# woolgathering/pyPeriod

Hardware: AMD Instinct MI355X
Metric: window-projections/sec (all-p sweep, N=4096) (higher is better)
Workload: dtype f64

## Files before the change

pyperiod_amd/csrc/period_hip.hip:

```cpp
#include <hip/hip_runtime.h>

#include <algorithm>
#include <cstdarg>
#include <cstdio>
#include <cstdlib>
#include <cstring>
#include <string>
#include <vector>

#include "../../include/periodhip.h"
#include "ph_kernels.h"
#include "ph_fit.h"
#include "ph_frames.h"

namespace {

thread_local std::string g_err;

int fail(int code, const char* fmt, ...) {
  char buf[512];
  va_list ap;
  va_start(ap, fmt);
  vsnprintf(buf, sizeof buf, fmt, ap);
  va_end(ap);
// ... 1391 lines not shown
  PH_TRY(st.out(B_OUT2, bases, (size_t)W * num * N * sz, &dbases));
  PH_TRY(st.out(B_OUT3, status, (size_t)W * sizeof(int32_t), &dstat));
  void* dsweeps;
  PH_TRY(st.out(B_OUT4, n_sweeps, (size_t)W * sizeof(int32_t), &dsweeps));
  PH_TRY(ensure(c, c->buf[B_WS0], (size_t)W * sizeof(double)));
  double* dnorm = static_cast<double*>(c->buf[B_WS0].p);
  const int row_stride = (max_length + 127) & ~127;
  PH_TRY(ensure(c, c->buf[B_WS1], (size_t)W * num * row_stride * sz));
  void* drows = c->buf[B_WS1].p;
  const unsigned kflags = flags & (PH_FLAG_TRUNC | PH_FLAG_ORTH);
  const int max_iters = 12 * (P + num) + 64;
  const dim3 grid((unsigned)W);
  if (pair) {
    PairWs ws;
    PH_TRY(pair_workspace(c, W, N, &ws));
    PH_TRY(launch(c, "k_mbest_step1", ph::k_mbest_step1_pair, dim3((unsigned)((W + 1) / 2)), s1.block, s1.lds,
                  (const double*)dx, (int)W, N, num, min_length, max_length, p_scr, gamma, tb.fac_off, tb.fac_q, geom, ws.geomf,
                  ws.radq, plan, n_pass, ws.gwin, max_iters, (uint32_t*)dper, (double*)dpow, (double*)drows, row_stride, dnorm,
                  (int*)dstat, (int*)dsweeps, c->pair_fold_once ? ph::pair_thin_band(N) : -1.0, c->pair_fold_report ? 1 : 0));
  } else {
    PH_TRY(dispatch(dtype, !gwin1, [&](auto t, auto lw) {
      using T = decltype(t);
      return launch(c, "k_mbest_step1", ph::k_mbest_step1<T, decltype(lw)::value>, grid, s1.block, s1.lds, (const T*)dx, N,
                    num, min_length, max_length, gamma, kflags, tb, geom, plan, n_pass, (T*)gbuf1, (T*)gwin1, max_iters,
                    (uint32_t*)dper, (double*)dpow, (T*)drows, row_stride, dnorm, (int*)dstat, (int*)dsweeps,
                    s1.small_means);
    }));
  }
  PH_TRY(dispatch(dtype, !gwin2, [&](auto t, auto lw) {
    using T = decltype(t);
    return launch(c, "k_mbest_step2", ph::k_mbest_step2<T, decltype(lw)::value>, grid, s2.block, s2.lds, N, num, gamma,
                  max_length, kflags, tb, geom, max_fac, (T*)gbuf2, (T*)gwin2, (uint32_t*)dper, (double*)dpow, (T*)dbases,
                  dnorm, (const int*)dstat, (T*)drows, row_stride);
  }));
// ... 1094 lines not shown
```

pyperiod_amd/csrc/ph_device.h:

```cpp
#pragma once

#include <hip/hip_runtime.h>
#include <stdint.h>

#include <type_traits>

namespace ph {

constexpr int kWave = 64;
constexpr int kBlock = 256;
constexpr int kBlockWide = 512;
constexpr int kMaxWaves = 16;
constexpr int kPairWaves = 16;

constexpr unsigned kTrunc = 1u;
constexpr unsigned kOrth = 2u;
constexpr unsigned kSingle = 4u;

struct Tables {
  const int* orth_off;
  const int* orth_q;
  const int* fac_off;
  const int* fac_q;
};
// ... 146 lines not shown
  a = uniform_f64(ta);
  b = uniform_f64(tb);
}

template <int NW = 0>
__device__ __forceinline__ double block_max(double v, double* red) {
  const int tid = threadIdx.x;
  const int nw = wave_count<NW>();
  v = wave_max(v);
  if ((tid & (kWave - 1)) == 0) red[tid >> 6] = v;
  __syncthreads();
  const double t = red_combine<true, NW>(red, nw);
  __syncthreads();
  return uniform_f64(t);
}

struct Fold {
  int p;
  int rows;
  int nfull;
  int trows;
  __device__ __forceinline__ Fold(int N, int p_) : p(p_) {
    rows = (N + p_ - 1) / p_;
    const int shortn = rows * p_ - N;
    nfull = p_ - shortn;
    trows = shortn == 0 ? rows : rows - 1;
  }
  __device__ __forceinline__ Fold(int p_, int rows_, int nfull_) : p(p_), rows(rows_), nfull(nfull_), trows(nfull_ == p_ ? rows_ : rows_ - 1) {}
  __device__ __forceinline__ int count(int j) const { return j < nfull ? rows : rows - 1; }
};
// ... 677 lines not shown
  take(v, p, dpp_f64<kDppRor8>(v), __builtin_amdgcn_update_dpp(0, p, kDppRor8, 0xF, 0xF, false));
  take(v, p, dpp_f64<kDppHalfMirror>(v), __builtin_amdgcn_update_dpp(0, p, kDppHalfMirror, 0xF, 0xF, false));
  take(v, p, dpp_f64<kDppXor2>(v), __builtin_amdgcn_update_dpp(0, p, kDppXor2, 0xF, 0xF, false));
  take(v, p, dpp_f64<kDppXor1>(v), __builtin_amdgcn_update_dpp(0, p, kDppXor1, 0xF, 0xF, false));
}

template <typename T>
__device__ __forceinline__ double block_sweep_value(const T* __restrict__ xs, T* __restrict__ buf, int N, int p,
                                                    int gamma_div, unsigned flags, const Tables& tb,
                                                    double* red) {
  project_lds(xs, buf, N, p, flags, tb);
  const double ss = block_sumsq(buf, N, red);
  return periodic_norm_from_sq(ss, N, gamma_div);
}

template <typename T>
__device__ __forceinline__ void zero_pad(T* __restrict__ xs, int N) {
  for (int i = threadIdx.x; i < kPad; i += blockDim.x) xs[N + i] = T(0);
}

template <typename T>
__device__ __forceinline__ void load_window(const T* __restrict__ g, T* __restrict__ xs, int N) {
  constexpr int V = 16 / sizeof(T);
  if ((reinterpret_cast<uintptr_t>(g) & 15) == 0 && (N % V) == 0) {
    using vec_t = typename std::conditional<sizeof(T) == 8, double2, float4>::type;
    const vec_t* gv = reinterpret_cast<const vec_t*>(g);
    vec_t* xv = reinterpret_cast<vec_t*>(xs);
    for (int i = threadIdx.x; i < N / V; i += blockDim.x) xv[i] = gv[i];
  } else {
    for (int i = threadIdx.x; i < N; i += blockDim.x) xs[i] = g[i];
  }
}

struct Carve {
  unsigned char* base;
  size_t off;
  __device__ explicit Carve(unsigned char* b) : base(b), off(0) {}
  template <typename U>
  __device__ U* take(size_t n) {
    U* p = reinterpret_cast<U*>(base + off);
    off += (n * sizeof(U) + 15) & ~size_t(15);
    return p;
  }
  __device__ Carve at(size_t o) const {
    Carve c(base);
// ... 113 lines not shown
```

pyperiod_amd/csrc/ph_mbest.h:

```cpp
#pragma once

#include "ph_device.h"
#include "ph_pair.h"

namespace ph {

__device__ __forceinline__ bool skip_test(const uint32_t* skip, int i) { return (skip[i >> 5] >> (i & 31)) & 1u; }
__device__ __forceinline__ void skip_set(uint32_t* skip, int i) { skip[i >> 5] |= 1u << (i & 31); }

template <typename Norm>
__device__ __forceinline__ bool mbest_prefers(double ss, int p, double best_ss, int bestp, int gamma, Norm&& norm) {
  bool take = bestp == 0;
  if (!take) {
    const double lhs = gamma ? ss * (double)bestp : ss;
    const double rhs = gamma ? best_ss * (double)p : best_ss;
    if (lhs > rhs * (1.0 + 1e-14)) {
      take = true;
    } else if (lhs >= rhs * (1.0 - 1e-14)) {
      const double vn = norm(ss, gamma ? p : 0);
      const double vb = norm(best_ss, gamma ? bestp : 0);
      take = vn > vb || (vn == vb && p < bestp);
    }
  }
  return take;
// ... 221 lines not shown
constexpr int kPairCoop = 6;

enum {
  MP_LISTED = 0,
  MP_FILLED = 2,
  MP_REPEATS = 4,
  MP_STATUS = 6,
  MP_SWEEPS = 8,
  MP_RUNNING = 10,
  MP_EXACT_ALL = 12,
  MP_QUEUE = 14,
  MP_WORDS = 16
};
enum { MP_UNIT = 0, MP_SCALE = 2, MP_DOUBLES = 4 };

__device__ __forceinline__ double pair_exact_part(const double* __restrict__ xs, int p, const PGeom& g, int first, int stride) {
  double part = 0.0;
  for (int j = first; j < p; j += stride) {
    const bool full = j < g.nfull;
    const double s = column_sum(xs, j, p, full ? g.rows : g.rows - 1);
    part = fma(s * s, full ? g.w_full : g.w_short, part);
  }
  return part;
}

struct Step1PairLds {
  f2* pw;
  double* stg;
  double* red;
  double* wbest;
  int* wbestp;
  double* norms;
  uint32_t* periods;
  uint32_t* skip;
  int* list;
  int* ctl;
  double* dst2;
  double* msm;
  double* prt;
  size_t bytes;
};
template <class C>
__host__ __device__ __forceinline__ Step1PairLds step1_pair_carve(C cv, int N, int num, int P) {
  Step1PairLds L;
  L.pw = cv.template take<f2>(N + kPad);
  L.stg = cv.template take<double>(N + kPad);
  L.red = cv.template take<double>(kRedDoubles);
  L.wbest = cv.template take<double>(kMaxWaves);
  L.wbestp = cv.template take<int>(kMaxWaves);
  L.norms = cv.template take<double>(2 * num);
  L.periods = cv.template take<uint32_t>(2 * num);
  L.skip = cv.template take<uint32_t>(2 * ((P + 31) / 32));
  L.list = cv.template take<int>(2 * kPairListCap);
  L.ctl = cv.template take<int>(MP_WORDS);
  L.dst2 = cv.template take<double>(MP_DOUBLES);
  L.msm = cv.template take<double>(kPairSmallP);
  L.prt = cv.template take<double>(kPairSplitW);
  L.bytes = cv.off;
  return L;
}

__global__ __launch_bounds__(1024) __attribute__((amdgpu_waves_per_eu(PH_STEP1_WAVES, 8))) void k_mbest_step1_pair(
    const double* __restrict__ x, int W, int N, int num, int p_lo, int p_hi, int p_scr, int gamma,
    const int* __restrict__ fac_off, const int* __restrict__ fac_q, const PGeom* __restrict__ geom, const PGeomF* __restrict__ geomf, const double* __restrict__ radq, const PassPlan* __restrict__ plan, int n_pass,
    double* __restrict__ gres, int max_iters, uint32_t* __restrict__ periods_out, double* __restrict__ norms_out,
    double* __restrict__ rows_out, int row_stride, double* __restrict__ dnorm_out, int* __restrict__ status_out,
    int* __restrict__ sweeps_out, double thin_band, int fold_report) {
  const bool fold_once = __double2hiint(thin_band) >= 0;
  extern __shared__ __attribute__((aligned(16))) unsigned char smem[];
  const int P = p_hi - p_lo + 1;
  const int SK = (P + 31) / 32;
  const Step1PairLds L = step1_pair_carve(Carve(smem), N, num, P);
  f2* pw = L.pw;
  double *stg = L.stg, *red = L.red, *wbest = L.wbest, *norms = L.norms, *dst2 = L.dst2, *msm = L.msm, *prt = L.prt;
  int *wbestp = L.wbestp, *list = L.list, *ctl = L.ctl;
  uint32_t *periods = L.periods, *skip = L.skip;

  const int tid = threadIdx.x;
  const int wv = __builtin_amdgcn_readfirstlane(tid >> 6);
  constexpr int NW = kPairWaves, nw = NW;
  const size_t gstride = win_stride((size_t)N);
  float* pwf = reinterpret_cast<float*>(pw);
  const double sqrtN = uniform_f64(sqrt((double)N));

  for (int k = tid; k < 2 * num; k += blockDim.x) {
    norms[k] = 0.0;
    periods[k] = 0u;
  }
  for (int k = tid; k < 2 * SK; k += blockDim.x) skip[k] = 0u;
  if (tid < MP_WORDS) ctl[tid] = tid == MP_QUEUE ? nw : 0;
  zero_pad(stg, N);
  for (int i = tid; i < kPad; i += blockDim.x) pw[N + i] = f2_zero();
  for (int w = 0; w < 2; ++w) {
    const int64_t gw = 2 * (int64_t)blockIdx.x + w;
    const bool exists = gw < W;
    __syncthreads();
    if (exists) {
      load_window(x + gw * (int64_t)N, stg, N);
    } else {
      for (int n = tid; n < N; n += blockDim.x) stg[n] = 0.0;
    }
    __syncthreads();
    const double rsq = block_sumsq<NW>(stg, N, red);
    const double sc = uniform_f64(pair_pick_scale(rsq, N));
    for (int n = tid; n < N; n += blockDim.x) pwf[2 * n + w] = (float)(stg[n] * sc);
    if (tid == 0) {
      dst2[MP_UNIT + w] = rsq * sc * sc * (1.0 + 1e-9);
      dst2[MP_SCALE + w] = sc;
      ctl[MP_RUNNING + w] = exists ? 1 : 0;
      ctl[MP_EXACT_ALL + w] = pair_usable(rsq) ? 0 : 1;
      if (exists) dnorm_out[gw] = periodic_norm_from_sq_n(rsq, sqrtN, 0);
    }
  }
  StageClock<kPairTimers, 6, 3> clk;
  WgStamp<kClocks> stamp;
  for (;;) {
    __syncthreads();
    const bool act0 = __builtin_amdgcn_readfirstlane(ctl[MP_RUNNING]) != 0, act1 = __builtin_amdgcn_readfirstlane(ctl[MP_RUNNING + 1]) != 0;
    if (!act0 && !act1) break;
    prio_by_progress(__builtin_amdgcn_readfirstlane(max(ctl[MP_SWEEPS], ctl[MP_SWEEPS + 1])));
    if (wv == 0 && pair_lane() == 0) ctl[MP_LISTED] = ctl[MP_LISTED + 1] = 0;
    f2* vals = reinterpret_cast<f2*>(stg);
    pair_sweep_plan<false, true>(
        pw, N, geomf, plan, wv, n_pass, nw, [&](float z, int q) { pair_store1(vals, z, q, p_lo); },
        [&](float z, int q_a, int q_b) { pair_store2(vals, z, q_a, q_b, p_lo); },
        PH_PAIR_QUEUE ? &ctl[MP_QUEUE] : nullptr);
    __syncthreads();
    clk.mark(0);
    prio_short_phase();
    {
    const int tid = (wv << 6) + pair_lane();
    const int lane = tid & (kWave - 1);
    if (tid == 0) ctl[MP_QUEUE] = nw;
    {
      const bool scr0 = act0 && !__builtin_amdgcn_readfirstlane(ctl[MP_EXACT_ALL]), scr1 = act1 && !__builtin_amdgcn_readfirstlane(ctl[MP_EXACT_ALL + 1]);
      if (scr0 || scr1) {
        const double unit0 = uniform_f64(dst2[MP_UNIT]), unit1 = uniform_f64(dst2[MP_UNIT + 1]);
        const int i0 = p_scr - p_lo;
        const bool cover = i0 > 0;
        const int SD = (i0 + 31) >> 5;
        uint32_t* seen = reinterpret_cast<uint32_t*>(stg);
        for (int k = tid; k < 2 * SD; k += blockDim.x) seen[k] = 0u;
        const double slack = cover ? pair_cover_slack(N) : 0.0;
        struct Entry {
          f2 v;
          double rad, rq;
          bool skip0, skip1;
        };
        auto entry = [&](int idx) {
          Entry e;
          const int q = p_lo + idx;
          const uint32_t bit = 1u << (idx & 31);
          e.v = vals[idx];
          e.rad = radq[q];
          e.rq = gamma ? 1.0 / (double)q : 1.0;
          e.skip0 = (skip[idx >> 5] & bit) != 0;
          e.skip1 = (skip[SK + (idx >> 5)] & bit) != 0;
          return e;
        };
        const int idx_own = i0 + tid;
        Entry own = {f2_zero(), 0.0, 1.0, true, true};
        if (idx_own < P) own = entry(idx_own);
        const double ninf = const_at_use(-1.0 / 0.0);
        double lo0 = ninf, lo1 = ninf;
        for (int idx = idx_own; idx < P; idx += blockDim.x) {
          const Entry e = idx == idx_own ? own : entry(idx);
          double a = (double)e.v.x - e.rad * unit0, b = (double)e.v.y - e.rad * unit1;
          if (gamma) {
            a *= e.rq;
            b *= e.rq;
          }
          if (!e.skip0 && a > lo0) lo0 = a;
          if (!e.skip1 && b > lo1) lo1 = b;
        }
        lo0 = wave_max(lo0);
        lo1 = wave_max(lo1);
        if (lane == 0) {
          red[wv] = lo0;
          red[kMaxWaves + wv] = lo1;
        }
        __syncthreads();
        lo0 = uniform_f64(red_combine<true, NW>(red, nw));
        lo1 = uniform_f64(red_combine<true, NW>(red + kMaxWaves, nw));
        const bool none0 = cover && scr0 && !(lo0 > ninf), none1 = cover && scr1 && !(lo1 > ninf);
        if (tid == 0 && none0) ctl[MP_LISTED] = kPairListCap + 1;
        if (tid == 0 && none1) ctl[MP_LISTED + 1] = kPairListCap + 1;
        const double thr0 = lo0 - fabs(lo0) * 1e-9, thr1 = lo1 - fabs(lo1) * 1e-9;
        for (int idx = idx_own; idx < P; idx += blockDim.x) {
          const Entry e = idx == idx_own ? own : entry(idx);
          const int q = p_lo + idx;
          const double rad = e.rad + slack;
          double a = (double)e.v.x + rad * unit0, b = (double)e.v.y + rad * unit1;
          if (gamma) {
            a *= e.rq;
            b *= e.rq;
          }
          const bool hit0 = scr0 && !none0 && a >= thr0, hit1 = scr1 && !none1 && b >= thr1;
          if (hit0 && !e.skip0) {
            const int k = atomicAdd(&ctl[MP_LISTED], 1);
            if (k < kPairListCap) list[k] = q;
          }
          if (hit1 && !e.skip1) {
            const int k = atomicAdd(&ctl[MP_LISTED + 1], 1);
// ... 9 lines not shown
              for (int w = 0; w < 2; ++w) {
                if (!(w ? hit1 : hit0) || (skip[w * SK + (di >> 5)] & dbit)) continue;
                if (atomicOr(&seen[w * SD + (di >> 5)], dbit) & dbit) continue;
                const int k = atomicAdd(&ctl[MP_LISTED + w], 1);
                if (k < kPairListCap) list[w * kPairListCap + k] = d;
              }
            }
          }
        }
      }
    }
    __syncthreads();
    clk.mark(1);
    for (int w = 0; w < 2; ++w) {
      if (!(w ? act1 : act0)) continue;
      const int64_t gw = 2 * (int64_t)blockIdx.x + w;
      int filled = __builtin_amdgcn_readfirstlane(ctl[MP_FILLED + w]), repeats = __builtin_amdgcn_readfirstlane(ctl[MP_REPEATS + w]), status = 0,
          iters = __builtin_amdgcn_readfirstlane(ctl[MP_SWEEPS + w]);
      const int nlisted = __builtin_amdgcn_readfirstlane(ctl[MP_LISTED + w]);
      const bool exact_all = __builtin_amdgcn_readfirstlane(ctl[MP_EXACT_ALL + w]) != 0 || nlisted > kPairListCap;
      int ncand = exact_all ? P : nlisted;
      double* nrm = norms + w * num;
      uint32_t* per = periods + w * num;
      uint32_t* sk = skip + w * SK;
      const int* lst = list + w * kPairListCap;
      __syncthreads();
      bool folded = false;
      if (iters + 1 > max_iters) {
        status = 2;
      } else {
// ... 6 lines not shown
          const int q0 = k0 < ncand ? lst[k0] : 0, q1 = k1 < ncand ? lst[k1] : 0;
          const unsigned long long t0 = __ballot(q0 >= p_scr), t1 = __ballot(q1 >= p_scr);
          if (__popcll(t0) + __popcll(t1) == 1) {
            const int m = t0 ? __builtin_amdgcn_readlane(q0, __builtin_amdgcn_readfirstlane(__ffsll((long long)t0) - 1))
                             : __builtin_amdgcn_readlane(q1, __builtin_amdgcn_readfirstlane(__ffsll((long long)t1) - 1));
            const float fm = (float)m;
            const int c0 = (int)(fm * __builtin_amdgcn_rcpf((float)max(q0, 1)) + 0.5f), c1 = (int)(fm * __builtin_amdgcn_rcpf((float)max(q1, 1)) + 0.5f);
            const bool odd = (k0 < ncand && c0 * q0 != m) || (k1 < ncand && c1 * q1 != m);
            if (m > kPairSmallP && __ballot(odd) == 0ull) fold_m = m;
          }
        }
        if (fold_m != 0) {
          const PGeom gm = geom[fold_m];
          double part = 0.0;
          if (tid == 0) wbestp[0] = 0;
          for (int j = tid; j < fold_m; j += blockDim.x) {
            const bool full = j < gm.nfull;
            const double s = pair_column_sum_global(src, j, fold_m, full ? gm.rows : gm.rows - 1);
            part = fma(s * s, full ? gm.w_full : gm.w_short, part);
            stg[j] = s;
          }
          fold_ss = block_sum<NW>(part, red);
          clk.mark(2);
          if (ncand > 1) {
            const int se = __builtin_amdgcn_frexp_exp(dst2[MP_SCALE + w]) - 1;
            const double band = thin_band * ldexp(dst2[MP_UNIT + w], -2 * se);
            double tie = 1e-9;
            asm volatile("" : "+s"(tie));
            const double thr = fold_ss - fabs(fold_ss) * tie - band;
            for (int k = wv; k < ncand; k += nw) {
              const int d = __builtin_amdgcn_readfirstlane(lst[k]);
              if (d == fold_m) continue;
              const double t = wave_sum(pair_thin_part(stg, fold_m, d, geom[d], lane));
              if (lane == 0 && !(t < thr)) wbestp[0] = 1;
            }
            __syncthreads();
            if (__builtin_amdgcn_readfirstlane(wbestp[0]) != 0) fold_m = 0;
          }
          clk.mark(3);
        }
        if (fold_m == 0) {
        load_window(src, stg, N);
        __syncthreads();
        clk.mark(2);
        if (p_scr > p_lo && !exact_all && ncand > 1) {
          for (int k = wv; k < ncand; k += nw) {
            const int p = lst[k];
            const PGeom g = geom[p];
            const double part = p < 64 ? wave_partial_small(stg, N, p, g, lane) : pair_exact_part(stg, p, g, lane, kWave);
            const double ss = wave_sum(part);
            if (lane == 0) msm[k] = ss;
          }
          __syncthreads();
          if (wv == 0) {
            const int k0 = lane, k1 = kWave + lane;
            const double v0 = k0 < ncand ? msm[k0] : -1.0, v1 = k1 < ncand ? msm[k1] : -1.0;
            const int q0 = lst[k0], q1 = k1 < kPairListCap ? lst[k1] : 0;
// ... 21 lines not shown
          clk.count(2, fold_m != 0 ? 1 : 0);
        }
        double best_ss = 0.0;
        int bestp = 0;
        const auto norm = [&](double s, int div) { return periodic_norm_from_sq_n(s, sqrtN, div); };
        auto consider = [&](double ss, int p) {
          if (!(ss > 0.0)) return;
          if (mbest_prefers(ss, p, best_ss, bestp, gamma, norm)) {
            best_ss = ss;
            bestp = p;
          }
        };
        double best = 0.0;
        if (fold_m != 0) {
          consider(fold_ss, fold_m);
          best = bestp != 0 ? periodic_norm_from_sq_n(best_ss, sqrtN, gamma ? bestp : 0) : 0.0;
          if (!(best > 0.0)) bestp = 0;
        } else if (ncand <= kPairCoop) {
          for (int k = 0; k < ncand; ++k) {
            const int p = exact_all ? p_lo + k : lst[k];
            if (skip_test(sk, p - p_lo)) continue;
            const PGeom g = geom[p];
            double part = 0.0;
            if (p < 64) {
              if (wv == 0) part = wave_partial_small(stg, N, p, g, lane);
            } else {
              part = pair_exact_part(stg, p, g, tid, blockDim.x);
            }
            consider(block_sum<NW>(part, red), p);
          }
          best = bestp != 0 ? periodic_norm_from_sq_n(best_ss, sqrtN, gamma ? bestp : 0) : 0.0;
          if (!(best > 0.0)) bestp = 0;
        } else {
          for (int k = wv; k < ncand; k += nw) {
            const int p = exact_all ? p_lo + k : lst[k];
            if (skip_test(sk, p - p_lo)) continue;
            const PGeom g = geom[p];
            const double part = p < 64 ? wave_partial_small(stg, N, p, g, lane) : pair_exact_part(stg, p, g, lane, kWave);
            consider(wave_sum(part), p);
          }
          best = bestp != 0 ? periodic_norm_from_sq_n(best_ss, sqrtN, gamma ? bestp : 0) : 0.0;
          if (!(best > 0.0)) bestp = 0;
// ... 11 lines not shown
        } else {
          int row = -1;
          for (int k0 = 0; k0 < num; k0 += kWave) {
            const unsigned long long hit = __ballot(k0 + lane < num && per[k0 + lane] == (uint32_t)bestp);
            if (hit) row = k0 + 63 - __clzll(hit);
          }
          const int action = mbest_book(row, bestp, best, p_lo, tid, filled, repeats, nrm, per, sk);
          double* brow = rows_out + (gw * (int64_t)num + (row < 0 ? 0 : row)) * row_stride;
          const bool more = filled < num;
          const double sc = uniform_f64(dst2[MP_SCALE + w]);
          double* dst = gres + gw * gstride;
          double acc = 0.0;
          const PGeom gb = geom[__builtin_amdgcn_readfirstlane(bestp)];
          const Fold f(bestp, gb.rows, gb.nfull);
          if (fold_m != 0) {
            for (int j = tid; j < bestp; j += blockDim.x) {
              const int cnt = f.count(j);
              const double m = stg[j] / (double)cnt;
              if (action == 1)
                brow[j] = m;
              else if (action == 2)
                brow[j] += m;
              if (more) {
                for (int r0 = 0; r0 < cnt; r0 += 4) {
                  const unsigned at = (unsigned)(r0 * bestp + j);
                  double v[4];
#pragma unroll
                  for (int u = 0; u < 4; ++u) v[u] = src[r0 + u < cnt ? at + (unsigned)(u * bestp) : at];
#pragma unroll
                  for (int u = 0; u < 4; ++u) {
                    if (r0 + u < cnt) {
// ... 6 lines not shown
                  }
                }
              }
            }
          } else if (bestp <= kPairSmallP) {
            split_row_means(stg, msm, prt, N, bestp, tid, kPairSplitW);
            if (tid < bestp) {
              const double m = msm[tid];
              if (action == 1)
                brow[tid] = m;
              else if (action == 2)
                brow[tid] += m;
            }
            if (more) {
              int idx = tid % bestp;
              const int step = blockDim.x % bestp;
              for (int n = tid; n < N; n += blockDim.x) {
                const double v = stg[n] - msm[idx];
                dst[n] = v;
                pwf[2 * n + w] = (float)(v * sc);
                acc = fma(v, v, acc);
                idx += step;
                idx = idx >= bestp ? idx - bestp : idx;
              }
            }
          } else {
            for (int j = tid; j < bestp; j += blockDim.x) {
              const double m = residue_mean(stg, f, j, false);
              const int cnt = f.count(j);
              if (action == 1)
                brow[j] = m;
              else if (action == 2)
                brow[j] += m;
              if (more) {
                for (int r = 0; r < cnt; ++r) {
                  const int n = r * bestp + j;
                  const double v = stg[n] - m;
                  dst[n] = v;
                  pwf[2 * n + w] = (float)(v * sc);
                  acc = fma(v, v, acc);
                }
              }
            }
          }
          if (more) {
            const double rsq = block_sum<NW>(acc, red);
            const double unit = rsq * sc * sc;
            const bool ok = rsq > 0.0 && rsq < const_at_use(1.79e308);
            if (ok && unit < const_at_use(kPairStaleMeanSq) * (double)const_at_use(N)) {
              const double sc2 = uniform_f64(pair_pick_scale(rsq, N));
              __syncthreads();
              pair_rescale(pwf, w, N, (float)(sc2 / sc), tid);
              if (tid == 0) {
                dst2[MP_UNIT + w] = rsq * sc2 * sc2 * (1.0 + 1e-9);
                dst2[MP_SCALE + w] = sc2;
              }
            } else if (tid == 0) {
              dst2[MP_UNIT + w] = unit * (1.0 + 1e-9);
            }
            if (tid == 0) ctl[MP_EXACT_ALL + w] = ok ? 0 : 1;
          }
        }
      }
      __syncthreads();
      if (tid == 0) {
        ctl[MP_FILLED + w] = filled;
        ctl[MP_REPEATS + w] = repeats;
        ctl[MP_STATUS + w] = status | (((ctl[MP_STATUS + w] >> 8) + (folded ? 1 : 0)) << 8);
        ctl[MP_SWEEPS + w] = iters;
        ctl[MP_RUNNING + w] = (status == 0 && filled < num) ? 1 : 0;
      }
      clk.mark(5);
    }
    }
  }
  if (kClocks && (blockIdx.x % 16) == 7 && tid == 0) {
    stamp.finish();
    printf("PAIRWG %d start %lld end %lld cycles %lld MHz %.0f hwid %x xcc %x\n", (int)blockIdx.x, stamp.wk0, stamp.wk1, stamp.ck1 - stamp.ck0,
           100.0 * (double)(stamp.ck1 - stamp.ck0) / (double)(stamp.wk1 - stamp.wk0), stamp.hwid, stamp.xcc);
  }
  if (kPairTimers && blockIdx.x < PH_PAIR_TIMERS_WGS && tid == 0)
    printf("pair timers (100 MHz ticks) screen %lld scan %lld load %lld thin %lld exact %lld update %lld  candidates %d exact_all %d folded %d sweeps %d %d\n",
           clk.ticks(0), clk.ticks(1), clk.ticks(2), clk.ticks(3), clk.ticks(4), clk.ticks(5), clk.counted(0), clk.counted(1), clk.counted(2), ctl[MP_SWEEPS],
           ctl[MP_SWEEPS + 1]);
  __syncthreads();
  for (int w = 0; w < 2; ++w) {
    const int64_t gw = 2 * (int64_t)blockIdx.x + w;
    if (gw >= W) continue;
    for (int k = tid; k < num; k += blockDim.x) {
      periods_out[gw * num + k] = periods[w * num + k];
      norms_out[gw * num + k] = norms[w * num + k];
    }
    if (tid == 0) {
      status_out[gw] = ctl[MP_STATUS + w] & 255;
      if (sweeps_out) sweeps_out[gw] = ctl[MP_SWEEPS + w] | (fold_report ? (ctl[MP_STATUS + w] >> 8) << 16 : 0);
    }
  }
}

__device__ __forceinline__ PGeom make_geom(int N, int p) {
  const int rows = (N + p - 1) / p;
  PGeom g;
  g.rows = rows;
  g.nfull = p - (rows * p - N);
  g.w_full = 1.0 / (double)rows;
  g.w_short = rows > 1 ? 1.0 / (double)(rows - 1) : 0.0;
  return g;
}

constexpr int kStep2Pre = 3;
// ... 281 lines not shown
```

pyperiod_amd/csrc/ph_pair.h:

```cpp
#pragma once

#include "ph_device.h"

namespace ph {

typedef float f2 __attribute__((ext_vector_type(2)));
typedef const volatile __attribute__((address_space(3))) f2* pair_ptr;

struct PGeomF {
  int rows;
  int nfull;
  float w_full;
  float w_short;
};

__device__ __forceinline__ f2 f2_make(float a, float b) {
  f2 r;
  r.x = a;
  r.y = b;
  return r;
}
__device__ __forceinline__ f2 f2_zero() { return f2_make(0.0f, 0.0f); }
__device__ __forceinline__ f2 f2_fma(f2 a, f2 b, f2 c) { return __builtin_elementwise_fma(a, b, c); }
__device__ __forceinline__ f2 f2_max(f2 a, f2 b) { return __builtin_elementwise_max(a, b); }
template <bool MX>
__device__ __forceinline__ f2 f2_acc(f2 part, f2 t) {
  return MX ? f2_max(part, t * t) : f2_fma(t, t, part);
}

template <int CTRL>
__device__ __forceinline__ f2 dpp_f2(f2 v) {
  const int a = __builtin_amdgcn_update_dpp(0, __float_as_int(v.x), CTRL, 0xF, 0xF, false);
  const int b = __builtin_amdgcn_update_dpp(0, __float_as_int(v.y), CTRL, 0xF, 0xF, false);
  return f2_make(__int_as_float(a), __int_as_float(b));
}

__device__ __forceinline__ int pair_lane() {
// ... 351 lines not shown
    const int whole = min(cut >> 6, last);
    const pair_ptr at = pair_at(xs);
    const int rem = whole & (UA - 1);
    if (UA > 3 && rem == 3) c = pair_duo_front<R, UA, (UA > 3 ? 3 : 1)>(at, q, pend, sa, pa, sb, pb);
    else if (UA > 2 && rem == 2) c = pair_duo_front<R, UA, (UA > 2 ? 2 : 1)>(at, q, pend, sa, pa, sb, pb);
    else if (rem == 1) c = pair_duo_front<R, UA, 1>(at, q, pend, sa, pa, sb, pb);
    else c = pair_duo_front<R, UA, UA>(at, q, pend, sa, pa, sb, pb);
    if constexpr (R <= 4) {
      for (; c + 2 * UA <= whole; c += 2 * UA) {
        pair_duo_group<R, R, UA, 0>(at + 64 * c, q, pend, sa, pa, sb, pb);
        pair_duo_group<R, R, UA, 0>(at + 64 * c + 64 * UA, q, pend, sa, pa, sb, pb);
      }
    }
    for (; c + UA <= whole; c += UA) pair_duo_group<R, R, UA, 0>(at + 64 * c, q, pend, sa, pa, sb, pb);
  }
  sb = pb = f2_zero();
  const unsigned long inq = pair_lanes_below(q - 64 * last);
  if (c < last && 64 * c < cut) {
    asm volatile("" ::: "memory");
    pair_duo_edge<R, R>(pair_at(xs) + 64 * c, q, pair_lanes_below(cut - 64 * c), ~0ul, pend, sa, pa, sb, pb);
    c += 1;
  }
  {
    const pair_ptr at = pair_at(xs);
    for (; c + 2 * UB <= last; c += 2 * UB) {
      pair_duo_group<R, R - 1, UB, 0>(at + 64 * c, q, pend, sa, pa, sb, pb);
      pair_duo_group<R, R - 1, UB, 0>(at + 64 * c + 64 * UB, q, pend, sa, pa, sb, pb);
    }
    for (; c + UB <= last; c += UB) pair_duo_group<R, R - 1, UB, 0>(at + 64 * c, q, pend, sa, pa, sb, pb);
    const int rem = last - c;
    if (rem > 0) {
// ... 21 lines not shown
  base = partner = f2_zero();
  switch (g.rows) {
#define PH_DUO_CASE(R)                                \
  case R:                                             \
    pair_duo_rows<R>(xs, N, q, g, base, partner);     \
    break;
    PH_DUO_CASE(3)
    PH_DUO_CASE(4)
    PH_DUO_CASE(5)
    PH_DUO_CASE(6)
#undef PH_DUO_CASE
    default: break;
  }
}

template <int M, bool MX = false>
__device__ __forceinline__ void pair_pass_multi(const f2* __restrict__ xs, int p, const PGeomF* __restrict__ geom,
                                                f2 (&total)[3]) {
  static_assert(M == 2 || M == 4, "two or four classes");
  const PGeomF g1 = geom[p], g2 = geom[2 * p], g4 = geom[(M == 4 ? 4 : 2) * p];
  const int lane = pair_lane();
  const int cut = g1.nfull;
  const int acols = min(p, (cut + 63) & ~63), rest = p - acols;
  const pair_ptr a = (pair_ptr)xs + lane;
  float wa[7], wb[7];
  wa[0] = g1.w_full;
  wb[0] = g1.w_short;
  wa[1] = g2.w_full;
  wa[3] = g4.w_full;
  if (!MX) {
    wa[2] = scalar_select_lt(p, g2.nfull, g2.w_full, g2.w_short);
#pragma unroll
// ... 105 lines not shown
  if ((l & 15) == 0) reinterpret_cast<float*>(vals)[2 * ((l < 32 ? qa : qb) - q0) + ((l >> 4) & 1)] = z;
}

__device__ __forceinline__ f2 pair_shift_down(f2 v, int lane, int by) {
  const int addr = ((lane + by) & (kWave - 1)) << 2;
  return f2_make(__int_as_float(__builtin_amdgcn_ds_bpermute(addr, __float_as_int(v.x))),
                 __int_as_float(__builtin_amdgcn_ds_bpermute(addr, __float_as_int(v.y))));
}

template <bool MX>
__device__ __forceinline__ f2 pair_chain_term(f2 tot, int lane, int q, const PGeomF& g) {
  const float w = MX ? 1.0f : (lane < g.nfull) ? g.w_full : g.w_short;
  return (lane < q) ? tot * tot * w : f2_zero();
}

template <bool MX, typename F, typename F2>
__device__ __forceinline__ void pair_chain_small(const f2* __restrict__ xs, int N, int L, int nlev,
                                                 const PGeomF* __restrict__ geom, F&& consume, F2&& consume2) {
  const int lane = pair_lane();
  PGeomF g = geom[L];
  const int full = g.nfull == L ? g.rows : g.rows - 1;
  const bool on = lane < L;
  const f2* ptr = xs + (on ? lane : 0);
  f2 s0 = f2_zero(), s1 = f2_zero();
  int r = 0;
  for (; r + 4 <= full; r += 4) {
    const f2 a = ptr[0], b = ptr[L], c = ptr[2 * L], d = ptr[3 * L];
    s0 += a;
    s1 += b;
    s0 += c;
    s1 += d;
    ptr += 4 * L;
  }
// ... 13 lines not shown
      const PGeomF g2 = geom[q2];
      tot += pair_shift_down(tot, lane, q2);
      const f2 vb = pair_chain_term<MX>(tot, lane, q2, g2);
      consume2(pair_reduce2<MX>(va, vb), q, q2);
      if (lev + 2 < nlev) {
        q = q2 >> 1;
        g = geom[q];
        tot += pair_shift_down(tot, lane, q);
      }
    } else {
      consume(pair_reduce1<MX>(va), q);
    }
  }
}

template <bool MX = false, bool DUO = false, typename F, typename F2>
__device__ __forceinline__ void pair_sweep_plan(const f2* __restrict__ xs, int N, const PGeomF* __restrict__ geom,
                                                const PassPlan* __restrict__ plan, int i_first, int i_end, int stride,
                                                F&& consume, F2&& consume2, int* __restrict__ queue = nullptr) {
  auto red = [](f2 v) { return pair_reduce1<MX>(v); };
  for (int i = i_first; i < i_end;) {
    int ticket = 0;
    if (queue && pair_lane() == 0) ticket = lds_ticket(queue);
    const int p = plan[i].p, m = plan[i].m;
    if (m >= 8) {
      pair_chain_small<MX>(xs, N, p, m - 8, geom, consume, consume2);
    } else if (m == 0) {
      consume(red(pair_partial_small<MX>(xs, N, p, geom[p])), p);
    } else if (m == 1) {
      consume(red(pair_pass_single<MX>(xs, p, geom[p])), p);
    } else if (DUO && m == 3) {
      f2 va, vb;
      pair_pass_duo(xs, N, p, geom[p], va, vb);
// ... 82 lines not shown

__device__ __forceinline__ bool pair_usable(double rsq) { return rsq > 0.0 && rsq < 1.79e308; }

__device__ __forceinline__ double pair_pick_scale(double rsq, int N) {
  if (!pair_usable(rsq)) return 1.0;
  int e;
  (void)frexp(rsq / (double)N, &e);
  return ldexp(1.0, -(e >> 1));
}

constexpr double kPairStaleMeanSq = 9.0e-13;
__device__ __forceinline__ bool pair_image_stale(double rsq, double sc, int N) {
  return pair_usable(rsq) && rsq * sc * sc < kPairStaleMeanSq * (double)N;
}

__device__ __forceinline__ void pair_rescale(float* __restrict__ pwf, int w, int N, float up, int tid = threadIdx.x) {
  for (int n = tid; n < N; n += blockDim.x) pwf[2 * n + w] *= up;
}

__device__ __forceinline__ int pair_rows_upper(float fn, int q) {
  return (int)(fn * __builtin_amdgcn_rcpf((float)q) * 1.000001f) + 1;
}

}
```

Measured before the change: 10.51 billion.

## Rematerialize pair-kernel args from kernarg segment to cut SGPR/VGPR pressure

```diff
diff --git a/pyperiod_amd/csrc/period_hip.hip b/pyperiod_amd/csrc/period_hip.hip
--- a/pyperiod_amd/csrc/period_hip.hip
+++ b/pyperiod_amd/csrc/period_hip.hip
@@ -1429,10 +1429,34 @@
   if (pair) {
     PairWs ws;
     PH_TRY(pair_workspace(c, W, N, &ws));
-    PH_TRY(launch(c, "k_mbest_step1", ph::k_mbest_step1_pair, dim3((unsigned)((W + 1) / 2)), s1.block, s1.lds,
-                  (const double*)dx, (int)W, N, num, min_length, max_length, p_scr, gamma, tb.fac_off, tb.fac_q, geom, ws.geomf,
-                  ws.radq, plan, n_pass, ws.gwin, max_iters, (uint32_t*)dper, (double*)dpow, (double*)drows, row_stride, dnorm,
-                  (int*)dstat, (int*)dsweeps, c->pair_fold_once ? ph::pair_thin_band(N) : -1.0, c->pair_fold_report ? 1 : 0));
+    ph::Step1PairArgs a;
+    a.x = (const double*)dx;
+    a.W = (int)W;
+    a.N = N;
+    a.num = num;
+    a.p_lo = min_length;
+    a.p_hi = max_length;
+    a.p_scr = p_scr;
+    a.gamma = gamma;
+    a.n_pass = n_pass;
+    a.fac_off = tb.fac_off;
+    a.fac_q = tb.fac_q;
+    a.geom = geom;
+    a.geomf = ws.geomf;
+    a.radq = ws.radq;
+    a.plan = plan;
+    a.gres = ws.gwin;
+    a.periods_out = (uint32_t*)dper;
+    a.norms_out = (double*)dpow;
+    a.rows_out = (double*)drows;
+    a.dnorm_out = dnorm;
+    a.status_out = (int*)dstat;
+    a.sweeps_out = (int*)dsweeps;
+    a.thin_band = c->pair_fold_once ? ph::pair_thin_band(N) : -1.0;
+    a.max_iters = max_iters;
+    a.row_stride = row_stride;
+    a.fold_report = c->pair_fold_report ? 1 : 0;
+    PH_TRY(launch(c, "k_mbest_step1", ph::k_mbest_step1_pair, dim3((unsigned)((W + 1) / 2)), s1.block, s1.lds, a));
   } else {
     PH_TRY(dispatch(dtype, !gwin1, [&](auto t, auto lw) {
       using T = decltype(t);
diff --git a/pyperiod_amd/csrc/ph_device.h b/pyperiod_amd/csrc/ph_device.h
--- a/pyperiod_amd/csrc/ph_device.h
+++ b/pyperiod_amd/csrc/ph_device.h
@@ -184,6 +184,22 @@
   __syncthreads();
   return uniform_f64(t);
 }
+
+template <typename T>
+struct ConstTable {
+  static_assert(sizeof(T) % 4 == 0, "entries are read word by word");
+  const __attribute__((address_space(4))) uint32_t* w;
+  __device__ __forceinline__ explicit ConstTable(const T* p) : w((const __attribute__((address_space(4))) uint32_t*)p) {}
+  __device__ __forceinline__ T operator[](int i) const {
+    constexpr int K = sizeof(T) / 4;
+    struct Words {
+      uint32_t v[K];
+    } r;
+#pragma unroll
+    for (int k = 0; k < K; ++k) r.v[k] = w[(int64_t)i * K + k];
+    return __builtin_bit_cast(T, r);
+  }
+};
 
 struct Fold {
   int p;
@@ -891,21 +907,21 @@
   return periodic_norm_from_sq(ss, N, gamma_div);
 }
 
-template <typename T>
+template <int NW = 0, typename T>
 __device__ __forceinline__ void zero_pad(T* __restrict__ xs, int N) {
-  for (int i = threadIdx.x; i < kPad; i += blockDim.x) xs[N + i] = T(0);
-}
-
-template <typename T>
+  for (int i = threadIdx.x; i < kPad; i += block_threads<NW>()) xs[N + i] = T(0);
+}
+
+template <int NW = 0, typename T>
 __device__ __forceinline__ void load_window(const T* __restrict__ g, T* __restrict__ xs, int N) {
   constexpr int V = 16 / sizeof(T);
   if ((reinterpret_cast<uintptr_t>(g) & 15) == 0 && (N % V) == 0) {
     using vec_t = typename std::conditional<sizeof(T) == 8, double2, float4>::type;
     const vec_t* gv = reinterpret_cast<const vec_t*>(g);
     vec_t* xv = reinterpret_cast<vec_t*>(xs);
-    for (int i = threadIdx.x; i < N / V; i += blockDim.x) xv[i] = gv[i];
+    for (int i = threadIdx.x; i < N / V; i += block_threads<NW>()) xv[i] = gv[i];
   } else {
-    for (int i = threadIdx.x; i < N; i += blockDim.x) xs[i] = g[i];
+    for (int i = threadIdx.x; i < N; i += block_threads<NW>()) xs[i] = g[i];
   }
 }
 
diff --git a/pyperiod_amd/csrc/ph_mbest.h b/pyperiod_amd/csrc/ph_mbest.h
--- a/pyperiod_amd/csrc/ph_mbest.h
+++ b/pyperiod_amd/csrc/ph_mbest.h
@@ -259,6 +259,21 @@
 };
 enum { MP_UNIT = 0, MP_SCALE = 2, MP_DOUBLES = 4 };
 
+template <int NW>
+__device__ __forceinline__ double block_sum_lead(double v, double* red, int wv, int lane) {
+  static_assert(kRedDoubles > kMaxWaves, "the total lies behind the partial sums");
+  double* total = red + kMaxWaves;
+  v = wave_sum(v);
+  if (lane == 0) red[wv] = v;
+  __syncthreads();
+  if (wv == 0) {
+    const double t = red_combine<false, NW>(red, NW);
+    if (lane == 0) *total = t;
+  }
+  __syncthreads();
+  return uniform_f64(*total);
+}
+
 __device__ __forceinline__ double pair_exact_part(const double* __restrict__ xs, int p, const PGeom& g, int first, int stride) {
   double part = 0.0;
   for (int j = first; j < p; j += stride) {
@@ -288,6 +303,8 @@
 template <class C>
 __host__ __device__ __forceinline__ Step1PairLds step1_pair_carve(C cv, int N, int num, int P) {
   Step1PairLds L;
+  L.ctl = cv.template take<int>(MP_WORDS);
+  L.dst2 = cv.template take<double>(MP_DOUBLES);
   L.pw = cv.template take<f2>(N + kPad);
   L.stg = cv.template take<double>(N + kPad);
   L.red = cv.template take<double>(kRedDoubles);
@@ -297,95 +314,148 @@
   L.periods = cv.template take<uint32_t>(2 * num);
   L.skip = cv.template take<uint32_t>(2 * ((P + 31) / 32));
   L.list = cv.template take<int>(2 * kPairListCap);
-  L.ctl = cv.template take<int>(MP_WORDS);
-  L.dst2 = cv.template take<double>(MP_DOUBLES);
   L.msm = cv.template take<double>(kPairSmallP);
   L.prt = cv.template take<double>(kPairSplitW);
   L.bytes = cv.off;
   return L;
 }
 
-__global__ __launch_bounds__(1024) __attribute__((amdgpu_waves_per_eu(PH_STEP1_WAVES, 8))) void k_mbest_step1_pair(
-    const double* __restrict__ x, int W, int N, int num, int p_lo, int p_hi, int p_scr, int gamma,
-    const int* __restrict__ fac_off, const int* __restrict__ fac_q, const PGeom* __restrict__ geom, const PGeomF* __restrict__ geomf, const double* __restrict__ radq, const PassPlan* __restrict__ plan, int n_pass,
-    double* __restrict__ gres, int max_iters, uint32_t* __restrict__ periods_out, double* __restrict__ norms_out,
-    double* __restrict__ rows_out, int row_stride, double* __restrict__ dnorm_out, int* __restrict__ status_out,
-    int* __restrict__ sweeps_out, double thin_band, int fold_report) {
-  const bool fold_once = __double2hiint(thin_band) >= 0;
+struct Step1PairArgs {
+  const double* x;
+  int W, N, num, p_lo, p_hi, p_scr, gamma;
+  int n_pass;
+  const int* fac_off;
+  const int* fac_q;
+  const PGeom* geom;
+  const PGeomF* geomf;
+  const double* radq;
+  const PassPlan* plan;
+  double* gres;
+  uint32_t* periods_out;
+  double* norms_out;
+  double* rows_out;
+  double* dnorm_out;
+  int* status_out;
+  int* sweeps_out;
+  double thin_band;
+  int max_iters, row_stride, fold_report;
+};
+typedef const __attribute__((address_space(4))) Step1PairArgs* step1_pair_args_ptr;
+
+__device__ __forceinline__ step1_pair_args_ptr pair_args_at_use() {
+  step1_pair_args_ptr p = (step1_pair_args_ptr)__builtin_amdgcn_kernarg_segment_ptr();
+  asm volatile("" : "+s"(p));
+  return p;
+}
+__device__ __forceinline__ Step1PairLds pair_lds_at_use(step1_pair_args_ptr A, unsigned char* smem) {
+  return step1_pair_carve(Carve(smem), A->N, A->num, A->p_hi - A->p_lo + 1);
+}
+template <typename T>
+__device__ __forceinline__ T* pair_arg_global(T* p) {
+  return (T*)(__attribute__((address_space(1))) T*)p;
+}
+template <typename T>
+__device__ __forceinline__ ConstTable<T> pair_arg_table(const T* p) {
+  return ConstTable<T>(p);
+}
+
+__global__ __launch_bounds__(1024) __attribute__((amdgpu_waves_per_eu(PH_STEP1_WAVES, 8))) void k_mbest_step1_pair(const Step1PairArgs) {
+  const step1_pair_args_ptr a = (step1_pair_args_ptr)__builtin_amdgcn_kernarg_segment_ptr();
+  const int scr_N = a->N, scr_p_lo = a->p_lo, scr_n_pass = a->n_pass;
+  const ConstTable<PGeomF> scr_geomf = pair_arg_table(a->geomf);
+  const ConstTable<PassPlan> scr_plan = pair_arg_table(a->plan);
   extern __shared__ __attribute__((aligned(16))) unsigned char smem[];
-  const int P = p_hi - p_lo + 1;
-  const int SK = (P + 31) / 32;
-  const Step1PairLds L = step1_pair_carve(Carve(smem), N, num, P);
-  f2* pw = L.pw;
-  double *stg = L.stg, *red = L.red, *wbest = L.wbest, *norms = L.norms, *dst2 = L.dst2, *msm = L.msm, *prt = L.prt;
-  int *wbestp = L.wbestp, *list = L.list, *ctl = L.ctl;
+  const Step1PairLds scr_L = pair_lds_at_use(a, smem);
+  f2* scr_pw = scr_L.pw;
+  double* scr_stg = scr_L.stg;
+  int* scr_ctl = scr_L.ctl;
+
+  const int tid = threadIdx.x;
+  const int scr_wv = __builtin_amdgcn_readfirstlane(tid >> 6);
+  constexpr int NW = kPairWaves, nw = NW;
+  constexpr int kThreads = NW * kWave;
+  const double sqrtN = uniform_f64(sqrt((double)scr_N));
+
+  {
+  const int N = scr_N, p_lo = scr_p_lo;
+  const Step1PairLds& L = scr_L;
+  f2* pw = scr_pw;
+  double* stg = scr_stg;
+  int* ctl = scr_ctl;
+  const int SK = (a->p_hi - p_lo + 1 + 31) / 32;
+  double *red = L.red, *norms = L.norms, *dst2 = L.dst2;
   uint32_t *periods = L.periods, *skip = L.skip;
-
-  const int tid = threadIdx.x;
-  const int wv = __builtin_amdgcn_readfirstlane(tid >> 6);
-  constexpr int NW = kPairWaves, nw = NW;
-  const size_t gstride = win_stride((size_t)N);
   float* pwf = reinterpret_cast<float*>(pw);
-  const double sqrtN = uniform_f64(sqrt((double)N));
-
-  for (int k = tid; k < 2 * num; k += blockDim.x) {
+  for (int k = tid; k < 2 * a->num; k += kThreads) {
     norms[k] = 0.0;
     periods[k] = 0u;
   }
-  for (int k = tid; k < 2 * SK; k += blockDim.x) skip[k] = 0u;
+  for (int k = tid; k < 2 * SK; k += kThreads) skip[k] = 0u;
   if (tid < MP_WORDS) ctl[tid] = tid == MP_QUEUE ? nw : 0;
-  zero_pad(stg, N);
-  for (int i = tid; i < kPad; i += blockDim.x) pw[N + i] = f2_zero();
+  zero_pad<NW>(stg, N);
+  for (int i = tid; i < kPad; i += kThreads) pw[N + i] = f2_zero();
   for (int w = 0; w < 2; ++w) {
     const int64_t gw = 2 * (int64_t)blockIdx.x + w;
-    const bool exists = gw < W;
+    const bool exists = gw < a->W;
     __syncthreads();
     if (exists) {
-      load_window(x + gw * (int64_t)N, stg, N);
+      load_window<NW>(pair_arg_global(a->x) + gw * (int64_t)N, stg, N);
     } else {
-      for (int n = tid; n < N; n += blockDim.x) stg[n] = 0.0;
+      for (int n = tid; n < N; n += kThreads) stg[n] = 0.0;
     }
     __syncthreads();
     const double rsq = block_sumsq<NW>(stg, N, red);
     const double sc = uniform_f64(pair_pick_scale(rsq, N));
-    for (int n = tid; n < N; n += blockDim.x) pwf[2 * n + w] = (float)(stg[n] * sc);
+    for (int n = tid; n < N; n += kThreads) pwf[2 * n + w] = (float)(stg[n] * sc);
     if (tid == 0) {
       dst2[MP_UNIT + w] = rsq * sc * sc * (1.0 + 1e-9);
       dst2[MP_SCALE + w] = sc;
       ctl[MP_RUNNING + w] = exists ? 1 : 0;
       ctl[MP_EXACT_ALL + w] = pair_usable(rsq) ? 0 : 1;
-      if (exists) dnorm_out[gw] = periodic_norm_from_sq_n(rsq, sqrtN, 0);
-    }
+      if (exists) pair_arg_global(a->dnorm_out)[gw] = periodic_norm_from_sq_n(rsq, sqrtN, 0);
+    }
+  }
   }
   StageClock<kPairTimers, 6, 3> clk;
   WgStamp<kClocks> stamp;
   for (;;) {
     __syncthreads();
-    const bool act0 = __builtin_amdgcn_readfirstlane(ctl[MP_RUNNING]) != 0, act1 = __builtin_amdgcn_readfirstlane(ctl[MP_RUNNING + 1]) != 0;
+    const bool act0 = __builtin_amdgcn_readfirstlane(scr_ctl[MP_RUNNING]) != 0, act1 = __builtin_amdgcn_readfirstlane(scr_ctl[MP_RUNNING + 1]) != 0;
     if (!act0 && !act1) break;
-    prio_by_progress(__builtin_amdgcn_readfirstlane(max(ctl[MP_SWEEPS], ctl[MP_SWEEPS + 1])));
-    if (wv == 0 && pair_lane() == 0) ctl[MP_LISTED] = ctl[MP_LISTED + 1] = 0;
-    f2* vals = reinterpret_cast<f2*>(stg);
+    prio_by_progress(__builtin_amdgcn_readfirstlane(max(scr_ctl[MP_SWEEPS], scr_ctl[MP_SWEEPS + 1])));
+    if (scr_wv == 0 && pair_lane() == 0) scr_ctl[MP_LISTED] = scr_ctl[MP_LISTED + 1] = 0;
+    f2* vals = reinterpret_cast<f2*>(scr_stg);
     pair_sweep_plan<false, true>(
-        pw, N, geomf, plan, wv, n_pass, nw, [&](float z, int q) { pair_store1(vals, z, q, p_lo); },
-        [&](float z, int q_a, int q_b) { pair_store2(vals, z, q_a, q_b, p_lo); },
-        PH_PAIR_QUEUE ? &ctl[MP_QUEUE] : nullptr);
+        scr_pw, scr_N, scr_geomf, scr_plan, scr_wv, scr_n_pass, nw, [&](float z, int q) { pair_store1(vals, z, q, scr_p_lo); },
+        [&](float z, int q_a, int q_b) { pair_store2(vals, z, q_a, q_b, scr_p_lo); },
+        PH_PAIR_QUEUE ? &scr_ctl[MP_QUEUE] : nullptr);
     __syncthreads();
     clk.mark(0);
     prio_short_phase();
     {
+    const int wv = const_at_use(scr_wv);
     const int tid = (wv << 6) + pair_lane();
     const int lane = tid & (kWave - 1);
-    if (tid == 0) ctl[MP_QUEUE] = nw;
+    if (tid == 0) scr_ctl[MP_QUEUE] = nw;
     {
-      const bool scr0 = act0 && !__builtin_amdgcn_readfirstlane(ctl[MP_EXACT_ALL]), scr1 = act1 && !__builtin_amdgcn_readfirstlane(ctl[MP_EXACT_ALL + 1]);
+      const bool scr0 = act0 && !__builtin_amdgcn_readfirstlane(scr_ctl[MP_EXACT_ALL]), scr1 = act1 && !__builtin_amdgcn_readfirstlane(scr_ctl[MP_EXACT_ALL + 1]);
       if (scr0 || scr1) {
+        const step1_pair_args_ptr A = pair_args_at_use();
+        const int N = A->N, p_lo = A->p_lo, P = A->p_hi - p_lo + 1, SK = (P + 31) / 32, p_scr = A->p_scr, gamma = A->gamma;
+        const Step1PairLds L = pair_lds_at_use(A, smem);
+        double *stg = L.stg, *red = L.red, *dst2 = L.dst2;
+        int *list = L.list, *ctl = L.ctl;
+        const uint32_t* skip = L.skip;
+        const f2* vals = reinterpret_cast<const f2*>(stg);
+        const ConstTable<double> radq = pair_arg_table(A->radq);
+        const ConstTable<int> fac_off = pair_arg_table(A->fac_off);
+        const ConstTable<int> fac_q = pair_arg_table(A->fac_q);
         const double unit0 = uniform_f64(dst2[MP_UNIT]), unit1 = uniform_f64(dst2[MP_UNIT + 1]);
         const int i0 = p_scr - p_lo;
         const bool cover = i0 > 0;
         const int SD = (i0 + 31) >> 5;
         uint32_t* seen = reinterpret_cast<uint32_t*>(stg);
-        for (int k = tid; k < 2 * SD; k += blockDim.x) seen[k] = 0u;
+        for (int k = tid; k < 2 * SD; k += kThreads) seen[k] = 0u;
         const double slack = cover ? pair_cover_slack(N) : 0.0;
         struct Entry {
           f2 v;
@@ -408,7 +478,7 @@
         if (idx_own < P) own = entry(idx_own);
         const double ninf = const_at_use(-1.0 / 0.0);
         double lo0 = ninf, lo1 = ninf;
-        for (int idx = idx_own; idx < P; idx += blockDim.x) {
+        for (int idx = idx_own; idx < P; idx += kThreads) {
           const Entry e = idx == idx_own ? own : entry(idx);
           double a = (double)e.v.x - e.rad * unit0, b = (double)e.v.y - e.rad * unit1;
           if (gamma) {
@@ -431,7 +501,7 @@
         if (tid == 0 && none0) ctl[MP_LISTED] = kPairListCap + 1;
         if (tid == 0 && none1) ctl[MP_LISTED + 1] = kPairListCap + 1;
         const double thr0 = lo0 - fabs(lo0) * 1e-9, thr1 = lo1 - fabs(lo1) * 1e-9;
-        for (int idx = idx_own; idx < P; idx += blockDim.x) {
+        for (int idx = idx_own; idx < P; idx += kThreads) {
           const Entry e = idx == idx_own ? own : entry(idx);
           const int q = p_lo + idx;
           const double rad = e.rad + slack;
@@ -471,6 +541,20 @@
     clk.mark(1);
     for (int w = 0; w < 2; ++w) {
       if (!(w ? act1 : act0)) continue;
+      const step1_pair_args_ptr A = pair_args_at_use();
+      const int N = A->N, p_lo = A->p_lo, P = A->p_hi - p_lo + 1, SK = (P + 31) / 32;
+      const int num = A->num, p_scr = A->p_scr, gamma = A->gamma, max_iters = A->max_iters, row_stride = A->row_stride;
+      const Step1PairLds L = pair_lds_at_use(A, smem);
+      double *stg = L.stg, *red = L.red, *wbest = L.wbest, *norms = L.norms, *dst2 = L.dst2, *msm = L.msm, *prt = L.prt;
+      int *wbestp = L.wbestp, *list = L.list, *ctl = L.ctl;
+      uint32_t *periods = L.periods, *skip = L.skip;
+      float* pwf = reinterpret_cast<float*>(L.pw);
+      const size_t gstride = win_stride((size_t)N);
+      const bool fold_once = __double2hiint(A->thin_band) >= 0;
+      const double* __restrict__ x = pair_arg_global(A->x);
+      double* __restrict__ gres = pair_arg_global(A->gres);
+      double* __restrict__ rows_out = pair_arg_global(A->rows_out);
+      const ConstTable<PGeom> geom = pair_arg_table(A->geom);
       const int64_t gw = 2 * (int64_t)blockIdx.x + w;
       int filled = __builtin_amdgcn_readfirstlane(ctl[MP_FILLED + w]), repeats = __builtin_amdgcn_readfirstlane(ctl[MP_REPEATS + w]), status = 0,
           iters = __builtin_amdgcn_readfirstlane(ctl[MP_SWEEPS + w]);
@@ -507,17 +591,17 @@
           const PGeom gm = geom[fold_m];
           double part = 0.0;
           if (tid == 0) wbestp[0] = 0;
-          for (int j = tid; j < fold_m; j += blockDim.x) {
+          for (int j = tid; j < fold_m; j += kThreads) {
             const bool full = j < gm.nfull;
             const double s = pair_column_sum_global(src, j, fold_m, full ? gm.rows : gm.rows - 1);
             part = fma(s * s, full ? gm.w_full : gm.w_short, part);
             stg[j] = s;
           }
-          fold_ss = block_sum<NW>(part, red);
+          fold_ss = block_sum_lead<NW>(part, red, wv, lane);
           clk.mark(2);
           if (ncand > 1) {
             const int se = __builtin_amdgcn_frexp_exp(dst2[MP_SCALE + w]) - 1;
-            const double band = thin_band * ldexp(dst2[MP_UNIT + w], -2 * se);
+            const double band = A->thin_band * ldexp(dst2[MP_UNIT + w], -2 * se);
             double tie = 1e-9;
             asm volatile("" : "+s"(tie));
             const double thr = fold_ss - fabs(fold_ss) * tie - band;
@@ -533,7 +617,7 @@
           clk.mark(3);
         }
         if (fold_m == 0) {
-        load_window(src, stg, N);
+        load_window<NW>(src, stg, N);
         __syncthreads();
         clk.mark(2);
         if (p_scr > p_lo && !exact_all && ncand > 1) {
@@ -585,8 +669,7 @@
         double best = 0.0;
         if (fold_m != 0) {
           consider(fold_ss, fold_m);
-          best = bestp != 0 ? periodic_norm_from_sq_n(best_ss, sqrtN, gamma ? bestp : 0) : 0.0;
-          if (!(best > 0.0)) bestp = 0;
+          if (wv == 0) best = bestp != 0 ? periodic_norm_from_sq_n(best_ss, sqrtN, gamma ? bestp : 0) : 0.0;
         } else if (ncand <= kPairCoop) {
           for (int k = 0; k < ncand; ++k) {
             const int p = exact_all ? p_lo + k : lst[k];
@@ -596,7 +679,7 @@
             if (p < 64) {
               if (wv == 0) part = wave_partial_small(stg, N, p, g, lane);
             } else {
-              part = pair_exact_part(stg, p, g, tid, blockDim.x);
+              part = pair_exact_part(stg, p, g, tid, kThreads);
             }
             consider(block_sum<NW>(part, red), p);
           }
@@ -638,7 +721,7 @@
           const PGeom gb = geom[__builtin_amdgcn_readfirstlane(bestp)];
           const Fold f(bestp, gb.rows, gb.nfull);
           if (fold_m != 0) {
-            for (int j = tid; j < bestp; j += blockDim.x) {
+            for (int j = tid; j < bestp; j += kThreads) {
               const int cnt = f.count(j);
               const double m = stg[j] / (double)cnt;
               if (action == 1)
@@ -675,8 +758,8 @@
             }
             if (more) {
               int idx = tid % bestp;
-              const int step = blockDim.x % bestp;
-              for (int n = tid; n < N; n += blockDim.x) {
+              const int step = kThreads % bestp;
+              for (int n = tid; n < N; n += kThreads) {
                 const double v = stg[n] - msm[idx];
                 dst[n] = v;
                 pwf[2 * n + w] = (float)(v * sc);
@@ -686,7 +769,7 @@
               }
             }
           } else {
-            for (int j = tid; j < bestp; j += blockDim.x) {
+            for (int j = tid; j < bestp; j += kThreads) {
               const double m = residue_mean(stg, f, j, false);
               const int cnt = f.count(j);
               if (action == 1)
@@ -705,13 +788,13 @@
             }
           }
           if (more) {
-            const double rsq = block_sum<NW>(acc, red);
+            const double rsq = block_sum_lead<NW>(acc, red, wv, lane);
             const double unit = rsq * sc * sc;
             const bool ok = rsq > 0.0 && rsq < const_at_use(1.79e308);
             if (ok && unit < const_at_use(kPairStaleMeanSq) * (double)const_at_use(N)) {
               const double sc2 = uniform_f64(pair_pick_scale(rsq, N));
               __syncthreads();
-              pair_rescale(pwf, w, N, (float)(sc2 / sc), tid);
+              pair_rescale<NW>(pwf, w, N, (float)(sc2 / sc), tid);
               if (tid == 0) {
                 dst2[MP_UNIT + w] = rsq * sc2 * sc2 * (1.0 + 1e-9);
                 dst2[MP_SCALE + w] = sc2;
@@ -742,19 +825,31 @@
   }
   if (kPairTimers && blockIdx.x < PH_PAIR_TIMERS_WGS && tid == 0)
     printf("pair timers (100 MHz ticks) screen %lld scan %lld load %lld thin %lld exact %lld update %lld  candidates %d exact_all %d folded %d sweeps %d %d\n",
-           clk.ticks(0), clk.ticks(1), clk.ticks(2), clk.ticks(3), clk.ticks(4), clk.ticks(5), clk.counted(0), clk.counted(1), clk.counted(2), ctl[MP_SWEEPS],
-           ctl[MP_SWEEPS + 1]);
+           clk.ticks(0), clk.ticks(1), clk.ticks(2), clk.ticks(3), clk.ticks(4), clk.ticks(5), clk.counted(0), clk.counted(1), clk.counted(2), scr_ctl[MP_SWEEPS],
+           scr_ctl[MP_SWEEPS + 1]);
   __syncthreads();
-  for (int w = 0; w < 2; ++w) {
-    const int64_t gw = 2 * (int64_t)blockIdx.x + w;
-    if (gw >= W) continue;
-    for (int k = tid; k < num; k += blockDim.x) {
-      periods_out[gw * num + k] = periods[w * num + k];
-      norms_out[gw * num + k] = norms[w * num + k];
-    }
-    if (tid == 0) {
-      status_out[gw] = ctl[MP_STATUS + w] & 255;
-      if (sweeps_out) sweeps_out[gw] = ctl[MP_SWEEPS + w] | (fold_report ? (ctl[MP_STATUS + w] >> 8) << 16 : 0);
+  {
+    const step1_pair_args_ptr A = pair_args_at_use();
+    const int num = A->num, fold_report = A->fold_report;
+    const Step1PairLds L = pair_lds_at_use(A, smem);
+    const double* norms = L.norms;
+    const uint32_t* periods = L.periods;
+    const int* ctl = L.ctl;
+    uint32_t* __restrict__ periods_out = pair_arg_global(A->periods_out);
+    double* __restrict__ norms_out = pair_arg_global(A->norms_out);
+    int* __restrict__ status_out = pair_arg_global(A->status_out);
+    int* __restrict__ sweeps_out = pair_arg_global(A->sweeps_out);
+    for (int w = 0; w < 2; ++w) {
+      const int64_t gw = 2 * (int64_t)blockIdx.x + w;
+      if (gw >= A->W) continue;
+      for (int k = tid; k < num; k += kThreads) {
+        periods_out[gw * num + k] = periods[w * num + k];
+        norms_out[gw * num + k] = norms[w * num + k];
+      }
+      if (tid == 0) {
+        status_out[gw] = ctl[MP_STATUS + w] & 255;
+        if (sweeps_out) sweeps_out[gw] = ctl[MP_SWEEPS + w] | (fold_report ? (ctl[MP_STATUS + w] >> 8) << 16 : 0);
+      }
     }
   }
 }
diff --git a/pyperiod_amd/csrc/ph_pair.h b/pyperiod_amd/csrc/ph_pair.h
--- a/pyperiod_amd/csrc/ph_pair.h
+++ b/pyperiod_amd/csrc/ph_pair.h
@@ -21,6 +21,11 @@
   return r;
 }
 __device__ __forceinline__ f2 f2_zero() { return f2_make(0.0f, 0.0f); }
+__device__ __forceinline__ f2 f2_zero_at_use() {
+  f2 r;
+  asm volatile("v_mov_b64 %0, 0" : "=v"(r));
+  return r;
+}
 __device__ __forceinline__ f2 f2_fma(f2 a, f2 b, f2 c) { return __builtin_elementwise_fma(a, b, c); }
 __device__ __forceinline__ f2 f2_max(f2 a, f2 b) { return __builtin_elementwise_max(a, b); }
 template <bool MX>
@@ -402,7 +407,8 @@
     }
     for (; c + UA <= whole; c += UA) pair_duo_group<R, R, UA, 0>(at + 64 * c, q, pend, sa, pa, sb, pb);
   }
-  sb = pb = f2_zero();
+  sb = f2_zero_at_use();
+  pb = f2_zero_at_use();
   const unsigned long inq = pair_lanes_below(q - 64 * last);
   if (c < last && 64 * c < cut) {
     asm volatile("" ::: "memory");
@@ -454,8 +460,8 @@
   }
 }
 
-template <int M, bool MX = false>
-__device__ __forceinline__ void pair_pass_multi(const f2* __restrict__ xs, int p, const PGeomF* __restrict__ geom,
+template <int M, bool MX = false, typename GT>
+__device__ __forceinline__ void pair_pass_multi(const f2* __restrict__ xs, int p, GT geom,
                                                 f2 (&total)[3]) {
   static_assert(M == 2 || M == 4, "two or four classes");
   const PGeomF g1 = geom[p], g2 = geom[2 * p], g4 = geom[(M == 4 ? 4 : 2) * p];
@@ -591,9 +597,9 @@
   return (lane < q) ? tot * tot * w : f2_zero();
 }
 
-template <bool MX, typename F, typename F2>
+template <bool MX, typename GT, typename F, typename F2>
 __device__ __forceinline__ void pair_chain_small(const f2* __restrict__ xs, int N, int L, int nlev,
-                                                 const PGeomF* __restrict__ geom, F&& consume, F2&& consume2) {
+                                                 GT geom, F&& consume, F2&& consume2) {
   const int lane = pair_lane();
   PGeomF g = geom[L];
   const int full = g.nfull == L ? g.rows : g.rows - 1;
@@ -637,9 +643,9 @@
   }
 }
 
-template <bool MX = false, bool DUO = false, typename F, typename F2>
-__device__ __forceinline__ void pair_sweep_plan(const f2* __restrict__ xs, int N, const PGeomF* __restrict__ geom,
-                                                const PassPlan* __restrict__ plan, int i_first, int i_end, int stride,
+template <bool MX = false, bool DUO = false, typename GT, typename PT, typename F, typename F2>
+__device__ __forceinline__ void pair_sweep_plan(const f2* __restrict__ xs, int N, GT geom,
+                                                PT plan, int i_first, int i_end, int stride,
                                                 F&& consume, F2&& consume2, int* __restrict__ queue = nullptr) {
   auto red = [](f2 v) { return pair_reduce1<MX>(v); };
   for (int i = i_first; i < i_end;) {
@@ -752,8 +758,9 @@
   return pair_usable(rsq) && rsq * sc * sc < kPairStaleMeanSq * (double)N;
 }
 
+template <int NW = 0>
 __device__ __forceinline__ void pair_rescale(float* __restrict__ pwf, int w, int N, float up, int tid = threadIdx.x) {
-  for (int n = tid; n < N; n += blockDim.x) pwf[2 * n + w] *= up;
+  for (int n = tid; n < N; n += block_threads<NW>()) pwf[2 * n + w] *= up;
 }
 
 __device__ __forceinline__ int pair_rows_upper(float fn, int q) {
```

After: 10.79 billion (median of 6 runs). 2.6% higher.
